# naver/dust3r

Hardware: NVIDIA H100
Metric: image-pairs/sec (512x384, ViT-L/B+DPT) (higher is better)
Workload: dtype bf16

## Files before the change

### dust3r_b200/csrc/attention_wgmma.cu

```cuda
#include "d3r_common.cuh"
#include "sm90_ptx.cuh"
#include "elementwise.h"
#include "prof.h"
#include "pdl.cuh"

namespace d3r {
namespace attn {

namespace wg {

constexpr int BQ = 128, BK = 128, D = 64;
constexpr int kThreads = 384;
constexpr int kTileBytes = 128 * 64 * 2;
constexpr int kPBytes = 2 * 64 * 128 * 2;
template <bool P_SMEM>
struct Smem {
  static constexpr int kP = P_SMEM ? 2 * kPBytes : 0;
  static constexpr int kBytes = kTileBytes  + 2 * kTileBytes  + 2 * kTileBytes  + kP + 128  + 1024;
  static_assert(kBytes <= 227 * 1024, "shared memory of one CTA");
};

template <bool P_SMEM>
__global__ void __launch_bounds__(kThreads, 1)
attention_kernel(const __grid_constant__ CUtensorMap tmap_q, const __grid_constant__ CUtensorMap tmap_k,
                 const __grid_constant__ CUtensorMap tmap_v, __nv_bfloat16* __restrict__ out, long long ldo, int Nq, int Nk,
                 int heads, int total_tiles, float scale_log2) {
  extern __shared__ uint8_t smem_raw[];
  uint8_t* smem = reinterpret_cast<uint8_t*>((reinterpret_cast<uintptr_t>(smem_raw) + 1023) & ~uintptr_t(1023));
  uint8_t* s_q = smem;
  uint8_t* s_k = s_q + kTileBytes;
  uint8_t* s_v = s_k + 2 * kTileBytes;
  uint8_t* s_p = s_v + 2 * kTileBytes;
  uint64_t* bars = reinterpret_cast<uint64_t*>(s_p + Smem<P_SMEM>::kP);
  uint64_t* q_full = bars + 0;
  uint64_t* q_empty = bars + 1;
  uint64_t* k_full = bars + 2;
  uint64_t* k_empty = bars + 4;
  uint64_t* v_full = bars + 6;
  uint64_t* v_empty = bars + 8;

  const int warp = threadIdx.x >> 5, lane = threadIdx.x & 31;
  const int nq_tiles = (Nq + BQ - 1) / BQ;
  const int nblk = (Nk + BK - 1) / BK;
  auto tile_coords = [&](int t, int& q0, int& h, int& b) {
    q0 = (t % nq_tiles) * BQ;
    h = (t / nq_tiles) % heads;
    b = t / (nq_tiles * heads);
  };

  if (threadIdx.x == 0) {
    ptx::prefetch_tmap(&tmap_q);
    ptx::prefetch_tmap(&tmap_k);
    ptx::prefetch_tmap(&tmap_v);
    ptx::mbar_init(ptx::smem_u32(q_full), 1);
    ptx::mbar_init(ptx::smem_u32(q_empty), 8);
    for (int s = 0; s < 2; ++s) {
      ptx::mbar_init(ptx::smem_u32(&k_full[s]), 1);
      ptx::mbar_init(ptx::smem_u32(&k_empty[s]), 8);
      ptx::mbar_init(ptx::smem_u32(&v_full[s]), 1);
      ptx::mbar_init(ptx::smem_u32(&v_empty[s]), 8);
    }
    ptx::fence_barrier_init();
  }
  __syncthreads();
  pdl::sync_with_predecessor();

  if (warp < 4) {
    ptx::setmaxnreg_dec<24>();
    if (warp == 0 && ptx::elect_one()) {
      uint32_t g = 0, it = 0;
      for (int t = blockIdx.x; t < total_tiles; t += gridDim.x, ++it) {
        int q0, h, b;
        tile_coords(t, q0, h, b);
        ptx::mbar_wait(ptx::smem_u32(q_empty), (it & 1) ^ 1);
        ptx::mbar_arrive_expect_tx(ptx::smem_u32(q_full), kTileBytes);
        ptx::tma_load_3d(ptx::smem_u32(s_q), &tmap_q, ptx::smem_u32(q_full), h * D, q0, b);
        for (int j = 0; j < nblk; ++j, ++g) {
          const int st = g & 1;
          const uint32_t ph = (g >> 1) & 1;
          ptx::mbar_wait(ptx::smem_u32(&k_empty[st]), ph ^ 1);
          ptx::mbar_arrive_expect_tx(ptx::smem_u32(&k_full[st]), kTileBytes);
          ptx::tma_load_3d(ptx::smem_u32(s_k + st * kTileBytes), &tmap_k, ptx::smem_u32(&k_full[st]), h * D, j * BK, b);
          ptx::mbar_wait(ptx::smem_u32(&v_empty[st]), ph ^ 1);
          ptx::mbar_arrive_expect_tx(ptx::smem_u32(&v_full[st]), kTileBytes);
          ptx::tma_load_3d(ptx::smem_u32(s_v + st * kTileBytes), &tmap_v, ptx::smem_u32(&v_full[st]), h * D, j * BK, b);
        }
      }
    }
  } else {
    ptx::setmaxnreg_inc<240>();
    const int cw = (threadIdx.x >> 7) - 1;
    const int wq = warp & 3, q = lane & 3;
    uint8_t* s_pw = s_p + cw * kPBytes;
    uint32_t g = 0, it = 0;
    for (int t = blockIdx.x; t < total_tiles; t += gridDim.x, ++it) {
      int q0, h, b;
      tile_coords(t, q0, h, b);
      float m_run[2] = {-INFINITY, -INFINITY}, l_run[2] = {0.f, 0.f};
      float o[32];
#pragma unroll
      for (int i = 0; i < 32; ++i) o[i] = 0.f;
      ptx::mbar_wait(ptx::smem_u32(q_full), it & 1);
      const uint64_t dq = ptx::desc_kmajor_sw128(ptx::smem_u32(s_q + cw * 64 * 128));
      for (int j = 0; j < nblk; ++j, ++g) {
        const int st = g & 1;
        const uint32_t ph = (g >> 1) & 1;
        float s[64];
        ptx::mbar_wait(ptx::smem_u32(&k_full[st]), ph);
        const uint64_t dk = ptx::desc_kmajor_sw128(ptx::smem_u32(s_k + st * kTileBytes));
        ptx::wgmma_fence();
#pragma unroll
        for (int k = 0; k < D / 16; ++k) ptx::wgmma_m64n128k16_ss(s, dq + uint64_t(2 * k), dk + uint64_t(2 * k), k ? 1u : 0u);
        ptx::wgmma_commit();
        ptx::wgmma_wait<0>();
        ptx::reg_fence(s);
        if (lane == 0) {
          ptx::mbar_arrive(ptx::smem_u32(&k_empty[st]));
          if (j == nblk - 1) ptx::mbar_arrive(ptx::smem_u32(q_empty));
        }
        const int nvalid = Nk - j * BK;
        if (nvalid < BK) {
#pragma unroll
          for (int n = 0; n < 16; ++n)
#pragma unroll
            for (int e = 0; e < 2; ++e)
              if (8 * n + 2 * q + e >= nvalid) { s[4 * n + e] = -INFINITY; s[4 * n + 2 + e] = -INFINITY; }
        }
        float ms[2];
#pragma unroll
        for (int hh = 0; hh < 2; ++hh) {
          float mx = -INFINITY;
#pragma unroll
          for (int n = 0; n < 16; ++n) mx = fmaxf(mx, fmaxf(s[4 * n + 2 * hh], s[4 * n + 2 * hh + 1]));
          mx = fmaxf(mx, __shfl_xor_sync(0xffffffffu, mx, 1));
          mx = fmaxf(mx, __shfl_xor_sync(0xffffffffu, mx, 2));
          const float m_new = fmaxf(m_run[hh], mx);
          const float corr = ptx::ex2_approx((m_run[hh] - m_new) * scale_log2);
          m_run[hh] = m_new;
          l_run[hh] *= corr;
#pragma unroll
          for (int n = 0; n < 8; ++n) { o[4 * n + 2 * hh] *= corr; o[4 * n + 2 * hh + 1] *= corr; }
          ms[hh] = m_new * scale_log2;
        }
        uint32_t pk[32];
#pragma unroll
        for (int n = 0; n < 16; ++n)
#pragma unroll
          for (int hh = 0; hh < 2; ++hh) {
            const float p0 = ptx::ex2_approx(fmaf(s[4 * n + 2 * hh], scale_log2, -ms[hh]));
            const float p1 = ptx::ex2_approx(fmaf(s[4 * n + 2 * hh + 1], scale_log2, -ms[hh]));
            l_run[hh] += p0 + p1;
            pk[2 * n + hh] = pack_bf16x2(p0, p1);
          }
        ptx::mbar_wait(ptx::smem_u32(&v_full[st]), ph);
        const uint32_t sv = ptx::smem_u32(s_v + st * kTileBytes);
        if constexpr (P_SMEM) {
#pragma unroll
          for (int n = 0; n < 16; ++n)
#pragma unroll
            for (int hh = 0; hh < 2; ++hh) {
              const int r = wq * 16 + (lane >> 2) + 8 * hh;
              *reinterpret_cast<uint32_t*>(s_pw + (n >> 3) * (64 * 128) + r * 128 + (((n & 7) ^ (r & 7)) << 4) + 4 * q) = pk[2 * n + hh];
            }
          ptx::fence_proxy_async();
          asm volatile("bar.sync %0, 128;" ::"r"(1 + cw) : "memory");
          const uint32_t sp = ptx::smem_u32(s_pw);
          ptx::wgmma_fence();
#pragma unroll
          for (int kk = 0; kk < BK / 16; ++kk)
            ptx::wgmma_m64n64k16_ss_tb(o, ptx::desc_kmajor_sw128(sp + (kk >> 2) * (64 * 128)) + uint64_t(2 * (kk & 3)),
                                       ptx::desc_mnmajor_sw128(sv + kk * 16 * 128), 1u);
        } else {
          ptx::wgmma_fence();
#pragma unroll
          for (int kk = 0; kk < BK / 16; ++kk) ptx::wgmma_m64n64k16_rs_tb(o, pk + 4 * kk, ptx::desc_mnmajor_sw128(sv + kk * 16 * 128), 1u);
        }
        ptx::wgmma_commit();
        ptx::wgmma_wait<0>();
        ptx::reg_fence(o);
        if constexpr (P_SMEM) asm volatile("bar.sync %0, 128;" ::"r"(1 + cw) : "memory");
        if (lane == 0) ptx::mbar_arrive(ptx::smem_u32(&v_empty[st]));
      }
#pragma unroll
      for (int hh = 0; hh < 2; ++hh) {
        float l = l_run[hh];
        l += __shfl_xor_sync(0xffffffffu, l, 1);
        l += __shfl_xor_sync(0xffffffffu, l, 2);
        const float inv = 1.f / l;
        const int qrow = q0 + cw * 64 + wq * 16 + (lane >> 2) + 8 * hh;
        if (qrow < Nq) {
          __nv_bfloat16* orow = out + ((long long)b * Nq + qrow) * ldo + h * D + 2 * q;
#pragma unroll
          for (int n = 0; n < 8; ++n)
            *reinterpret_cast<uint32_t*>(orow + 8 * n) = pack_bf16x2(o[4 * n + 2 * hh] * inv, o[4 * n + 2 * hh + 1] * inv);
        }
      }
    }
  }
}

}

template <bool P_SMEM>
static int launch_attention(const CUtensorMap& mq, const CUtensorMap& mk, const CUtensorMap& mv, void* out, long long ldo, int B, int heads,
                            int Nq, int Nk, float scale, cudaStream_t st) {
  static unsigned long long attr_devices = 0;
  if (first_launch_on_this_device(attr_devices))
    D3R_CUDA(cudaFuncSetAttribute(wg::attention_kernel<P_SMEM>, cudaFuncAttributeMaxDynamicSharedMemorySize, wg::Smem<P_SMEM>::kBytes));
  const int total_tiles = ((Nq + wg::BQ - 1) / wg::BQ) * heads * B;
  const int slots = num_sms();
  const int rounds = (total_tiles + slots - 1) / slots;
  const int grid = (total_tiles + rounds - 1) / rounds;
  prof::Scope scope(P_SMEM ? "attention_wgmma_psmem" : "attention_wgmma", st, 4.0 * double(B) * heads * double(Nq) * double(Nk) * 64.0);
  D3R_CUDA(pdl::launch(wg::attention_kernel<P_SMEM>, dim3(grid), dim3(wg::kThreads), size_t(wg::Smem<P_SMEM>::kBytes), st, mq, mk, mv,
                       (__nv_bfloat16*)out, ldo, Nq, Nk, heads, total_tiles, scale * 1.4426950408889634f));
  D3R_LAUNCH_CHECK();
  return D3R_OK;
}

static int make_map(CUtensorMap* m, const void* base, long long ld, int cols, int N, int B, int box_rows) {
  const cuuint64_t dims[3] = {(cuuint64_t)cols, (cuuint64_t)N, (cuuint64_t)B};
  const cuuint64_t str[2] = {(cuuint64_t)ld * 2, (cuuint64_t)N * ld * 2};
  const cuuint32_t box[3] = {64, (cuuint32_t)box_rows, 1};
  return encode_tensor_map(m, base, 3, dims, str, box, "attention");
}

static int g_impl = 3;

int attention_hd64(const void* q, long long ldq, const void* k, long long ldk, const void* v, long long ldv, void* out,
                   long long ldo, int B, int heads, int Nq, int Nk, float scale, cudaStream_t st) {
  D3R_CHECK_ARG(q && k && v && out && B > 0 && heads > 0 && Nq > 0 && Nk > 0, "attention: bad arguments");
  D3R_CHECK_ARG(ldq % 8 == 0 && ldk % 8 == 0 && ldv % 8 == 0 && ldo % 8 == 0, "attention: row strides must be multiples of 8");
  D3R_CHECK_ARG(((uintptr_t)q & 15) == 0 && ((uintptr_t)k & 15) == 0 && ((uintptr_t)v & 15) == 0 && ((uintptr_t)out & 15) == 0,
                "attention: pointers must be 16-byte aligned");
  CUtensorMap mq, mk, mv;
  int rc;
  if ((rc = make_map(&mq, q, ldq, heads * 64, Nq, B, wg::BQ))) return rc;
  if ((rc = make_map(&mk, k, ldk, heads * 64, Nk, B, wg::BK))) return rc;
  if ((rc = make_map(&mv, v, ldv, heads * 64, Nk, B, wg::BK))) return rc;
  if (g_impl == 2) return launch_attention<true>(mq, mk, mv, out, ldo, B, heads, Nq, Nk, scale, st);
  return launch_attention<false>(mq, mk, mv, out, ldo, B, heads, Nq, Nk, scale, st);
}

}
}

extern "C" void d3r_set_attention_impl(int32_t impl) { d3r::attn::g_impl = (impl == 2) ? 2 : 3; }

extern "C" int d3r_attention_hd64(const void* q, int64_t ldq, const void* k, int64_t ldk, const void* v, int64_t ldv, void* out,
                                  int64_t ldo, int32_t B, int32_t heads, int32_t Nq, int32_t Nk, float scale, void* stream) {
  return d3r::attn::attention_hd64(q, ldq, k, ldk, v, ldv, out, ldo, B, heads, Nq, Nk, scale, (cudaStream_t)stream);
}
```

### dust3r_b200/csrc/sm90_ptx.cuh

```cuda
#pragma once
#include <cuda.h>
#include <cuda_runtime.h>
#include <cuda_bf16.h>
#include <cstdint>

namespace d3r {
namespace ptx {

__device__ __forceinline__ uint32_t smem_u32(const void* p) { return static_cast<uint32_t>(__cvta_generic_to_shared(p)); }

__device__ __forceinline__ bool elect_one() {
  uint32_t pred = 0;
  asm volatile(
      "{\n"
      ".reg .b32 %%rx;\n"
      ".reg .pred %%px;\n"
      "elect.sync %%rx|%%px, %1;\n"
      "@%%px mov.s32 %0, 1;\n"
      "}\n"
      : "+r"(pred)
      : "r"(0xffffffffu));
  return pred != 0;
}

__device__ __forceinline__ void mbar_init(uint32_t bar, uint32_t count) {
  asm volatile("mbarrier.init.shared::cta.b64 [%0], %1;" ::"r"(bar), "r"(count));
}
__device__ __forceinline__ void fence_barrier_init() { asm volatile("fence.mbarrier_init.release.cluster;" ::: "memory"); }
__device__ __forceinline__ void fence_proxy_async() { asm volatile("fence.proxy.async.shared::cta;" ::: "memory"); }

__device__ __forceinline__ void mbar_arrive_expect_tx(uint32_t bar, uint32_t bytes) {
  asm volatile("mbarrier.arrive.expect_tx.shared::cta.b64 _, [%0], %1;" ::"r"(bar), "r"(bytes) : "memory");
}
__device__ __forceinline__ void mbar_arrive(uint32_t bar) {
  asm volatile("mbarrier.arrive.shared::cta.b64 _, [%0];" ::"r"(bar) : "memory");
}
__device__ __forceinline__ bool mbar_try_wait(uint32_t bar, uint32_t parity) {
  uint32_t done;
  asm volatile(
      "{\n"
      ".reg .pred p;\n"
      "mbarrier.try_wait.parity.shared::cta.b64 p, [%1], %2;\n"
      "selp.u32 %0, 1, 0, p;\n"
      "}\n"
      : "=r"(done)
      : "r"(bar), "r"(parity)
      : "memory");
  return done != 0;
}
__device__ __forceinline__ void mbar_wait(uint32_t bar, uint32_t parity) {
  while (!mbar_try_wait(bar, parity)) {
  }
}
__device__ __forceinline__ void mbar_wait_bounded(uint32_t bar, uint32_t parity) {
  uint32_t spins = 0;
  bool done;
  do {
    done = mbar_try_wait(bar, parity);
    if (!done && ++spins > (1u << 22)) __trap();
  } while (!done);
}

__device__ __forceinline__ void bulk_g2s(uint32_t dst, const void* src, uint32_t bytes, uint32_t bar) {
  asm volatile("cp.async.bulk.shared::cluster.global.mbarrier::complete_tx::bytes [%0], [%1], %2, [%3];"
               ::"r"(dst), "l"(src), "r"(bytes), "r"(bar) : "memory");
}
__device__ __forceinline__ uint64_t policy_evict_first() {
  uint64_t pol;
  asm volatile("createpolicy.fractional.L2::evict_first.b64 %0, 1.0;" : "=l"(pol));
  return pol;
}
__device__ __forceinline__ void bulk_g2s_hint(uint32_t dst, const void* src, uint32_t bytes, uint32_t bar, uint64_t pol) {
  asm volatile("cp.async.bulk.shared::cluster.global.mbarrier::complete_tx::bytes.L2::cache_hint [%0], [%1], %2, [%3], %4;"
               ::"r"(dst), "l"(src), "r"(bytes), "r"(bar), "l"(pol) : "memory");
}

__device__ __forceinline__ void prefetch_tmap(const void* tmap) {
  asm volatile("prefetch.tensormap [%0];" ::"l"(reinterpret_cast<uint64_t>(tmap)) : "memory");
}
__device__ __forceinline__ void tma_load_2d(uint32_t dst, const void* tmap, uint32_t bar, int c0, int c1) {
  asm volatile(
      "cp.async.bulk.tensor.2d.shared::cluster.global.mbarrier::complete_tx::bytes [%0], [%1, {%3, %4}], [%2];"
      ::"r"(dst), "l"(reinterpret_cast<uint64_t>(tmap)), "r"(bar), "r"(c0), "r"(c1)
      : "memory");
}
__device__ __forceinline__ void tma_load_3d(uint32_t dst, const void* tmap, uint32_t bar, int c0, int c1, int c2) {
  asm volatile(
      "cp.async.bulk.tensor.3d.shared::cluster.global.mbarrier::complete_tx::bytes [%0], [%1, {%3, %4, %5}], [%2];"
      ::"r"(dst), "l"(reinterpret_cast<uint64_t>(tmap)), "r"(bar), "r"(c0), "r"(c1), "r"(c2)
      : "memory");
}
__device__ __forceinline__ void tma_load_4d(uint32_t dst, const void* tmap, uint32_t bar, int c0, int c1, int c2, int c3) {
  asm volatile(
      "cp.async.bulk.tensor.4d.shared::cluster.global.mbarrier::complete_tx::bytes [%0], [%1, {%3, %4, %5, %6}], [%2];"
      ::"r"(dst), "l"(reinterpret_cast<uint64_t>(tmap)), "r"(bar), "r"(c0), "r"(c1), "r"(c2), "r"(c3)
      : "memory");
}
__device__ __forceinline__ void tma_load_3d_mc(uint32_t dst, const void* tmap, uint32_t bar, int c0, int c1, int c2, uint16_t mask) {
  asm volatile(
      "cp.async.bulk.tensor.3d.shared::cluster.global.mbarrier::complete_tx::bytes.multicast::cluster [%0], [%1, {%3, %4, %5}], [%2], %6;"
      ::"r"(dst), "l"(reinterpret_cast<uint64_t>(tmap)), "r"(bar), "r"(c0), "r"(c1), "r"(c2), "h"(mask)
      : "memory");
}

__device__ __forceinline__ void tma_store_2d(const void* tmap, uint32_t src, int c0, int c1) {
  asm volatile("cp.async.bulk.tensor.2d.global.shared::cta.tile.bulk_group [%0, {%2, %3}], [%1];"
               ::"l"(reinterpret_cast<uint64_t>(tmap)), "r"(src), "r"(c0), "r"(c1) : "memory");
}
__device__ __forceinline__ void tma_store_4d(const void* tmap, uint32_t src, int c0, int c1, int c2, int c3) {
  asm volatile("cp.async.bulk.tensor.4d.global.shared::cta.tile.bulk_group [%0, {%2, %3, %4, %5}], [%1];"
               ::"l"(reinterpret_cast<uint64_t>(tmap)), "r"(src), "r"(c0), "r"(c1), "r"(c2), "r"(c3) : "memory");
}
__device__ __forceinline__ void tma_reduce_add_2d(const void* tmap, uint32_t src, int c0, int c1) {
  asm volatile("cp.reduce.async.bulk.tensor.2d.global.shared::cta.add.tile.bulk_group [%0, {%2, %3}], [%1];"
               ::"l"(reinterpret_cast<uint64_t>(tmap)), "r"(src), "r"(c0), "r"(c1) : "memory");
}
__device__ __forceinline__ void bulk_commit_group() { asm volatile("cp.async.bulk.commit_group;" ::: "memory"); }
template <int N> __device__ __forceinline__ void bulk_wait_group_read() { asm volatile("cp.async.bulk.wait_group.read %0;" ::"n"(N) : "memory"); }
template <int N> __device__ __forceinline__ void bulk_wait_group() { asm volatile("cp.async.bulk.wait_group %0;" ::"n"(N) : "memory"); }
__device__ __forceinline__ void st_shared_b32(uint32_t addr, uint32_t v) { asm volatile("st.shared.b32 [%0], %1;" ::"r"(addr), "r"(v) : "memory"); }
__device__ __forceinline__ uint32_t ld_shared_b32(uint32_t addr) {
  uint32_t v;
  asm volatile("ld.shared.b32 %0, [%1];" : "=r"(v) : "r"(addr) : "memory");
  return v;
}
__device__ __forceinline__ void st_shared_v2_f32(uint32_t addr, float a, float b) {
  asm volatile("st.shared.v2.f32 [%0], {%1, %2};" ::"r"(addr), "f"(a), "f"(b) : "memory");
}
__device__ __forceinline__ void named_bar_sync(uint32_t id, uint32_t count) { asm volatile("bar.sync %0, %1;" ::"r"(id), "r"(count) : "memory"); }

__device__ __forceinline__ uint32_t cluster_ctarank() {
  uint32_t r;
  asm volatile("mov.u32 %0, %%cluster_ctarank;" : "=r"(r));
  return r;
}
__device__ __forceinline__ void cluster_sync() {
  asm volatile("barrier.cluster.arrive.release.aligned;\nbarrier.cluster.wait.acquire.aligned;" ::: "memory");
}
__device__ __forceinline__ void mbar_arrive_cluster(uint32_t bar, uint32_t rank) {
  asm volatile(
      "{\n"
      ".reg .b32 raddr;\n"
      "mapa.shared::cluster.u32 raddr, %0, %1;\n"
      "mbarrier.arrive.shared::cluster.b64 _, [raddr];\n"
      "}\n" ::"r"(bar), "r"(rank) : "memory");
}

__device__ __forceinline__ float ex2_approx(float x) { float y; asm("ex2.approx.ftz.f32 %0, %1;" : "=f"(y) : "f"(x)); return y; }
__device__ __forceinline__ float rcp_approx(float x) { float y; asm("rcp.approx.ftz.f32 %0, %1;" : "=f"(y) : "f"(x)); return y; }
__device__ __forceinline__ float rsqrt_approx(float x) { float y; asm("rsqrt.approx.ftz.f32 %0, %1;" : "=f"(y) : "f"(x)); return y; }
__device__ __forceinline__ float sqrt_approx(float x) { float y; asm("sqrt.approx.ftz.f32 %0, %1;" : "=f"(y) : "f"(x)); return y; }

template <int N> __device__ __forceinline__ void setmaxnreg_dec() { asm volatile("setmaxnreg.dec.sync.aligned.u32 %0;" ::"n"(N)); }
template <int N> __device__ __forceinline__ void setmaxnreg_inc() { asm volatile("setmaxnreg.inc.sync.aligned.u32 %0;" ::"n"(N)); }

__device__ __forceinline__ void wgmma_fence() { asm volatile("wgmma.fence.sync.aligned;" ::: "memory"); }
__device__ __forceinline__ void wgmma_commit() { asm volatile("wgmma.commit_group.sync.aligned;" ::: "memory"); }
template <int N> __device__ __forceinline__ void wgmma_wait() { asm volatile("wgmma.wait_group.sync.aligned %0;" ::"n"(N) : "memory"); }
template <int N> __device__ __forceinline__ void reg_fence(float (&d)[N]) {
#pragma unroll
  for (int i = 0; i < N; ++i) asm volatile("" : "+f"(d[i])::"memory");
}

__device__ __forceinline__ uint64_t desc_sw128(uint32_t smem_addr, uint32_t lbo_bytes) {
  uint64_t d = 0;
  d |= uint64_t((smem_addr & 0x3FFFF) >> 4);
  d |= uint64_t(lbo_bytes >> 4) << 16;
  d |= uint64_t(1024 >> 4) << 32;
  d |= uint64_t(1) << 62;
  return d;
}
__device__ __forceinline__ uint64_t desc_kmajor_sw128(uint32_t smem_addr) { return desc_sw128(smem_addr, 16); }
__device__ __forceinline__ uint64_t desc_mnmajor_sw128(uint32_t smem_addr) { return desc_sw128(smem_addr, 1024); }

__device__ __forceinline__ void wgmma_m64n64k16_ss(float* d, uint64_t desc_a, uint64_t desc_b, uint32_t accumulate) {
  asm volatile(
      "{\n"
      ".reg .pred p;\n"
      "setp.ne.b32 p, %34, 0;\n"
      "wgmma.mma_async.sync.aligned.m64n64k16.f32.bf16.bf16 "
      "{%0, %1, %2, %3, %4, %5, %6, %7, %8, %9, %10, %11, %12, %13, %14, %15, %16, %17, %18, %19, %20, %21, %22, %23, %24, %25, %26, %27, %28, %29, %30, %31}, %32, %33, p, 1, 1, 0, 0;\n"
      "}\n"
      : "+f"(d[0]), "+f"(d[1]), "+f"(d[2]), "+f"(d[3]), "+f"(d[4]), "+f"(d[5]), "+f"(d[6]), "+f"(d[7]), "+f"(d[8]), "+f"(d[9]), "+f"(d[10]), "+f"(d[11]), "+f"(d[12]), "+f"(d[13]), "+f"(d[14]), "+f"(d[15]), "+f"(d[16]), "+f"(d[17]), "+f"(d[18]), "+f"(d[19]), "+f"(d[20]), "+f"(d[21]), "+f"(d[22]), "+f"(d[23]), "+f"(d[24]), "+f"(d[25]), "+f"(d[26]), "+f"(d[27]), "+f"(d[28]), "+f"(d[29]), "+f"(d[30]), "+f"(d[31])
      : "l"(desc_a), "l"(desc_b), "r"(accumulate));
}
__device__ __forceinline__ void wgmma_m64n128k16_ss(float* d, uint64_t desc_a, uint64_t desc_b, uint32_t accumulate) {
  asm volatile(
      "{\n"
      ".reg .pred p;\n"
      "setp.ne.b32 p, %66, 0;\n"
      "wgmma.mma_async.sync.aligned.m64n128k16.f32.bf16.bf16 "
      "{%0, %1, %2, %3, %4, %5, %6, %7, %8, %9, %10, %11, %12, %13, %14, %15, %16, %17, %18, %19, %20, %21, %22, %23, %24, %25, %26, %27, %28, %29, %30, %31, %32, %33, %34, %35, %36, %37, %38, %39, %40, %41, %42, %43, %44, %45, %46, %47, %48, %49, %50, %51, %52, %53, %54, %55, %56, %57, %58, %59, %60, %61, %62, %63}, %64, %65, p, 1, 1, 0, 0;\n"
      "}\n"
      : "+f"(d[0]), "+f"(d[1]), "+f"(d[2]), "+f"(d[3]), "+f"(d[4]), "+f"(d[5]), "+f"(d[6]), "+f"(d[7]), "+f"(d[8]), "+f"(d[9]), "+f"(d[10]), "+f"(d[11]), "+f"(d[12]), "+f"(d[13]), "+f"(d[14]), "+f"(d[15]), "+f"(d[16]), "+f"(d[17]), "+f"(d[18]), "+f"(d[19]), "+f"(d[20]), "+f"(d[21]), "+f"(d[22]), "+f"(d[23]), "+f"(d[24]), "+f"(d[25]), "+f"(d[26]), "+f"(d[27]), "+f"(d[28]), "+f"(d[29]), "+f"(d[30]), "+f"(d[31]), "+f"(d[32]), "+f"(d[33]), "+f"(d[34]), "+f"(d[35]), "+f"(d[36]), "+f"(d[37]), "+f"(d[38]), "+f"(d[39]), "+f"(d[40]), "+f"(d[41]), "+f"(d[42]), "+f"(d[43]), "+f"(d[44]), "+f"(d[45]), "+f"(d[46]), "+f"(d[47]), "+f"(d[48]), "+f"(d[49]), "+f"(d[50]), "+f"(d[51]), "+f"(d[52]), "+f"(d[53]), "+f"(d[54]), "+f"(d[55]), "+f"(d[56]), "+f"(d[57]), "+f"(d[58]), "+f"(d[59]), "+f"(d[60]), "+f"(d[61]), "+f"(d[62]), "+f"(d[63])
      : "l"(desc_a), "l"(desc_b), "r"(accumulate));
}
__device__ __forceinline__ void wgmma_m64n256k16_ss(float* d, uint64_t desc_a, uint64_t desc_b, uint32_t accumulate) {
  asm volatile(
      "{\n"
      ".reg .pred p;\n"
      "setp.ne.b32 p, %130, 0;\n"
      "wgmma.mma_async.sync.aligned.m64n256k16.f32.bf16.bf16 "
      "{%0, %1, %2, %3, %4, %5, %6, %7, %8, %9, %10, %11, %12, %13, %14, %15, %16, %17, %18, %19, %20, %21, %22, %23, %24, %25, %26, %27, %28, %29, %30, %31, %32, %33, %34, %35, %36, %37, %38, %39, %40, %41, %42, %43, %44, %45, %46, %47, %48, %49, %50, %51, %52, %53, %54, %55, %56, %57, %58, %59, %60, %61, %62, %63, %64, %65, %66, %67, %68, %69, %70, %71, %72, %73, %74, %75, %76, %77, %78, %79, %80, %81, %82, %83, %84, %85, %86, %87, %88, %89, %90, %91, %92, %93, %94, %95, %96, %97, %98, %99, %100, %101, %102, %103, %104, %105, %106, %107, %108, %109, %110, %111, %112, %113, %114, %115, %116, %117, %118, %119, %120, %121, %122, %123, %124, %125, %126, %127}, %128, %129, p, 1, 1, 0, 0;\n"
      "}\n"
      : "+f"(d[0]), "+f"(d[1]), "+f"(d[2]), "+f"(d[3]), "+f"(d[4]), "+f"(d[5]), "+f"(d[6]), "+f"(d[7]), "+f"(d[8]), "+f"(d[9]), "+f"(d[10]), "+f"(d[11]), "+f"(d[12]), "+f"(d[13]), "+f"(d[14]), "+f"(d[15]), "+f"(d[16]), "+f"(d[17]), "+f"(d[18]), "+f"(d[19]), "+f"(d[20]), "+f"(d[21]), "+f"(d[22]), "+f"(d[23]), "+f"(d[24]), "+f"(d[25]), "+f"(d[26]), "+f"(d[27]), "+f"(d[28]), "+f"(d[29]), "+f"(d[30]), "+f"(d[31]), "+f"(d[32]), "+f"(d[33]), "+f"(d[34]), "+f"(d[35]), "+f"(d[36]), "+f"(d[37]), "+f"(d[38]), "+f"(d[39]), "+f"(d[40]), "+f"(d[41]), "+f"(d[42]), "+f"(d[43]), "+f"(d[44]), "+f"(d[45]), "+f"(d[46]), "+f"(d[47]), "+f"(d[48]), "+f"(d[49]), "+f"(d[50]), "+f"(d[51]), "+f"(d[52]), "+f"(d[53]), "+f"(d[54]), "+f"(d[55]), "+f"(d[56]), "+f"(d[57]), "+f"(d[58]), "+f"(d[59]), "+f"(d[60]), "+f"(d[61]), "+f"(d[62]), "+f"(d[63]), "+f"(d[64]), "+f"(d[65]), "+f"(d[66]), "+f"(d[67]), "+f"(d[68]), "+f"(d[69]), "+f"(d[70]), "+f"(d[71]), "+f"(d[72]), "+f"(d[73]), "+f"(d[74]), "+f"(d[75]), "+f"(d[76]), "+f"(d[77]), "+f"(d[78]), "+f"(d[79]), "+f"(d[80]), "+f"(d[81]), "+f"(d[82]), "+f"(d[83]), "+f"(d[84]), "+f"(d[85]), "+f"(d[86]), "+f"(d[87]), "+f"(d[88]), "+f"(d[89]), "+f"(d[90]), "+f"(d[91]), "+f"(d[92]), "+f"(d[93]), "+f"(d[94]), "+f"(d[95]), "+f"(d[96]), "+f"(d[97]), "+f"(d[98]), "+f"(d[99]), "+f"(d[100]), "+f"(d[101]), "+f"(d[102]), "+f"(d[103]), "+f"(d[104]), "+f"(d[105]), "+f"(d[106]), "+f"(d[107]), "+f"(d[108]), "+f"(d[109]), "+f"(d[110]), "+f"(d[111]), "+f"(d[112]), "+f"(d[113]), "+f"(d[114]), "+f"(d[115]), "+f"(d[116]), "+f"(d[117]), "+f"(d[118]), "+f"(d[119]), "+f"(d[120]), "+f"(d[121]), "+f"(d[122]), "+f"(d[123]), "+f"(d[124]), "+f"(d[125]), "+f"(d[126]), "+f"(d[127])
      : "l"(desc_a), "l"(desc_b), "r"(accumulate));
}
__device__ __forceinline__ void wgmma_m64n64k16_rs_tb(float* d, const uint32_t* a, uint64_t desc_b, uint32_t accumulate) {
  asm volatile(
      "{\n"
      ".reg .pred p;\n"
      "setp.ne.b32 p, %37, 0;\n"
      "wgmma.mma_async.sync.aligned.m64n64k16.f32.bf16.bf16 "
      "{%0, %1, %2, %3, %4, %5, %6, %7, %8, %9, %10, %11, %12, %13, %14, %15, %16, %17, %18, %19, %20, %21, %22, %23, %24, %25, %26, %27, %28, %29, %30, %31}, {%32, %33, %34, %35}, %36, p, 1, 1, 1;\n"
      "}\n"
      : "+f"(d[0]), "+f"(d[1]), "+f"(d[2]), "+f"(d[3]), "+f"(d[4]), "+f"(d[5]), "+f"(d[6]), "+f"(d[7]), "+f"(d[8]), "+f"(d[9]), "+f"(d[10]), "+f"(d[11]), "+f"(d[12]), "+f"(d[13]), "+f"(d[14]), "+f"(d[15]), "+f"(d[16]), "+f"(d[17]), "+f"(d[18]), "+f"(d[19]), "+f"(d[20]), "+f"(d[21]), "+f"(d[22]), "+f"(d[23]), "+f"(d[24]), "+f"(d[25]), "+f"(d[26]), "+f"(d[27]), "+f"(d[28]), "+f"(d[29]), "+f"(d[30]), "+f"(d[31])
      : "r"(a[0]), "r"(a[1]), "r"(a[2]), "r"(a[3]), "l"(desc_b), "r"(accumulate));
}
__device__ __forceinline__ void wgmma_m64n64k16_ss_tb(float* d, uint64_t desc_a, uint64_t desc_b, uint32_t accumulate) {
  asm volatile(
      "{\n"
      ".reg .pred p;\n"
      "setp.ne.b32 p, %34, 0;\n"
      "wgmma.mma_async.sync.aligned.m64n64k16.f32.bf16.bf16 "
      "{%0, %1, %2, %3, %4, %5, %6, %7, %8, %9, %10, %11, %12, %13, %14, %15, %16, %17, %18, %19, %20, %21, %22, %23, %24, %25, %26, %27, %28, %29, %30, %31}, %32, %33, p, 1, 1, 0, 1;\n"
      "}\n"
      : "+f"(d[0]), "+f"(d[1]), "+f"(d[2]), "+f"(d[3]), "+f"(d[4]), "+f"(d[5]), "+f"(d[6]), "+f"(d[7]), "+f"(d[8]), "+f"(d[9]), "+f"(d[10]), "+f"(d[11]), "+f"(d[12]), "+f"(d[13]), "+f"(d[14]), "+f"(d[15]), "+f"(d[16]), "+f"(d[17]), "+f"(d[18]), "+f"(d[19]), "+f"(d[20]), "+f"(d[21]), "+f"(d[22]), "+f"(d[23]), "+f"(d[24]), "+f"(d[25]), "+f"(d[26]), "+f"(d[27]), "+f"(d[28]), "+f"(d[29]), "+f"(d[30]), "+f"(d[31])
      : "l"(desc_a), "l"(desc_b), "r"(accumulate));
}

}
}
```

Measured before the change: 232.8.

## Rewrite default attention kernel as FA3-style ping-pong with intra-warpgroup overlap

The default register-P attention path becomes a new kernel with one TMA producer warpgroup and three consumer warpgroups handling 192 query rows. It uses double-buffered Q slots and a 3-stage K/V ring. Consumers take turns issuing WGMMAs through named barriers, so one warpgroup's softmax overlaps another's tensor-core work. Within a warpgroup, the next block's QK^T is issued alongside the previous block's PV, so softmax also overlaps matmul. The cost is higher register pressure per consumer, a 192-row tile that changes tile counts and wave quantization, and more intricate barrier and phase logic.

Result: faster. 237.4 (median of 6 runs) (+2.0%).

```diff
diff --git a/dust3r_b200/csrc/attention_wgmma.cu b/dust3r_b200/csrc/attention_wgmma.cu
--- a/dust3r_b200/csrc/attention_wgmma.cu
+++ b/dust3r_b200/csrc/attention_wgmma.cu
@@ -13,25 +13,23 @@
 constexpr int kThreads = 384;
 constexpr int kTileBytes = 128 * 64 * 2;
 constexpr int kPBytes = 2 * 64 * 128 * 2;
-template <bool P_SMEM>
-struct Smem {
-  static constexpr int kP = P_SMEM ? 2 * kPBytes : 0;
-  static constexpr int kBytes = kTileBytes  + 2 * kTileBytes  + 2 * kTileBytes  + kP + 128  + 1024;
+
+struct SmemPsmem {
+  static constexpr int kBytes = kTileBytes  + 2 * kTileBytes  + 2 * kTileBytes  + 2 * kPBytes + 128  + 1024;
   static_assert(kBytes <= 227 * 1024, "shared memory of one CTA");
 };
 
-template <bool P_SMEM>
 __global__ void __launch_bounds__(kThreads, 1)
-attention_kernel(const __grid_constant__ CUtensorMap tmap_q, const __grid_constant__ CUtensorMap tmap_k,
-                 const __grid_constant__ CUtensorMap tmap_v, __nv_bfloat16* __restrict__ out, long long ldo, int Nq, int Nk,
-                 int heads, int total_tiles, float scale_log2) {
+attention_psmem_kernel(const __grid_constant__ CUtensorMap tmap_q, const __grid_constant__ CUtensorMap tmap_k,
+                       const __grid_constant__ CUtensorMap tmap_v, __nv_bfloat16* __restrict__ out, long long ldo, int Nq, int Nk,
+                       int heads, int total_tiles, float scale_log2) {
   extern __shared__ uint8_t smem_raw[];
   uint8_t* smem = reinterpret_cast<uint8_t*>((reinterpret_cast<uintptr_t>(smem_raw) + 1023) & ~uintptr_t(1023));
   uint8_t* s_q = smem;
   uint8_t* s_k = s_q + kTileBytes;
   uint8_t* s_v = s_k + 2 * kTileBytes;
   uint8_t* s_p = s_v + 2 * kTileBytes;
-  uint64_t* bars = reinterpret_cast<uint64_t*>(s_p + Smem<P_SMEM>::kP);
+  uint64_t* bars = reinterpret_cast<uint64_t*>(s_p + 2 * kPBytes);
   uint64_t* q_full = bars + 0;
   uint64_t* q_empty = bars + 1;
   uint64_t* k_full = bars + 2;
@@ -154,31 +152,25 @@
           }
         ptx::mbar_wait(ptx::smem_u32(&v_full[st]), ph);
         const uint32_t sv = ptx::smem_u32(s_v + st * kTileBytes);
-        if constexpr (P_SMEM) {
-#pragma unroll
-          for (int n = 0; n < 16; ++n)
-#pragma unroll
-            for (int hh = 0; hh < 2; ++hh) {
-              const int r = wq * 16 + (lane >> 2) + 8 * hh;
-              *reinterpret_cast<uint32_t*>(s_pw + (n >> 3) * (64 * 128) + r * 128 + (((n & 7) ^ (r & 7)) << 4) + 4 * q) = pk[2 * n + hh];
-            }
-          ptx::fence_proxy_async();
-          asm volatile("bar.sync %0, 128;" ::"r"(1 + cw) : "memory");
-          const uint32_t sp = ptx::smem_u32(s_pw);
-          ptx::wgmma_fence();
-#pragma unroll
-          for (int kk = 0; kk < BK / 16; ++kk)
-            ptx::wgmma_m64n64k16_ss_tb(o, ptx::desc_kmajor_sw128(sp + (kk >> 2) * (64 * 128)) + uint64_t(2 * (kk & 3)),
-                                       ptx::desc_mnmajor_sw128(sv + kk * 16 * 128), 1u);
-        } else {
-          ptx::wgmma_fence();
-#pragma unroll
-          for (int kk = 0; kk < BK / 16; ++kk) ptx::wgmma_m64n64k16_rs_tb(o, pk + 4 * kk, ptx::desc_mnmajor_sw128(sv + kk * 16 * 128), 1u);
-        }
+#pragma unroll
+        for (int n = 0; n < 16; ++n)
+#pragma unroll
+          for (int hh = 0; hh < 2; ++hh) {
+            const int r = wq * 16 + (lane >> 2) + 8 * hh;
+            *reinterpret_cast<uint32_t*>(s_pw + (n >> 3) * (64 * 128) + r * 128 + (((n & 7) ^ (r & 7)) << 4) + 4 * q) = pk[2 * n + hh];
+          }
+        ptx::fence_proxy_async();
+        asm volatile("bar.sync %0, 128;" ::"r"(1 + cw) : "memory");
+        const uint32_t sp = ptx::smem_u32(s_pw);
+        ptx::wgmma_fence();
+#pragma unroll
+        for (int kk = 0; kk < BK / 16; ++kk)
+          ptx::wgmma_m64n64k16_ss_tb(o, ptx::desc_kmajor_sw128(sp + (kk >> 2) * (64 * 128)) + uint64_t(2 * (kk & 3)),
+                                     ptx::desc_mnmajor_sw128(sv + kk * 16 * 128), 1u);
         ptx::wgmma_commit();
         ptx::wgmma_wait<0>();
         ptx::reg_fence(o);
-        if constexpr (P_SMEM) asm volatile("bar.sync %0, 128;" ::"r"(1 + cw) : "memory");
+        asm volatile("bar.sync %0, 128;" ::"r"(1 + cw) : "memory");
         if (lane == 0) ptx::mbar_arrive(ptx::smem_u32(&v_empty[st]));
       }
 #pragma unroll
@@ -199,20 +191,252 @@
   }
 }
 
+constexpr int kConsumers = 3, kQRows = 64 * kConsumers, kPpThreads = 128 * (1 + kConsumers);
+constexpr int kQTileBytes = kQRows * 128;
+constexpr int kQSlots = 2, kKvStages = 3;
+constexpr int kBarTurn = 3;
+struct Smem {
+  static constexpr int kBytes = kQSlots * kQTileBytes + 2 * kKvStages * kTileBytes  + 128  + 1024;
+  static_assert(kBytes <= 227 * 1024, "shared memory of one CTA");
+};
+
+__global__ void __launch_bounds__(kPpThreads, 1)
+attention_kernel(const __grid_constant__ CUtensorMap tmap_q, const __grid_constant__ CUtensorMap tmap_k,
+                 const __grid_constant__ CUtensorMap tmap_v, __nv_bfloat16* __restrict__ out, long long ldo, int Nq, int Nk,
+                 int heads, int total_tiles, float scale_log2) {
+  extern __shared__ uint8_t smem_raw[];
+  uint8_t* smem = reinterpret_cast<uint8_t*>((reinterpret_cast<uintptr_t>(smem_raw) + 1023) & ~uintptr_t(1023));
+  uint8_t* s_q = smem;
+  uint8_t* s_k = s_q + kQSlots * kQTileBytes;
+  uint8_t* s_v = s_k + kKvStages * kTileBytes;
+  uint64_t* bars = reinterpret_cast<uint64_t*>(s_v + kKvStages * kTileBytes);
+  uint64_t* q_full = bars + 0;
+  uint64_t* q_empty = q_full + kQSlots;
+  uint64_t* k_full = q_empty + kQSlots;
+  uint64_t* k_empty = k_full + kKvStages;
+  uint64_t* v_full = k_empty + kKvStages;
+  uint64_t* v_empty = v_full + kKvStages;
+  auto slot = [](uint32_t u, uint32_t n) { return u % n; };
+  auto parity = [](uint32_t u, uint32_t n) { return (u / n) & 1u; };
+
+  const int warp = threadIdx.x >> 5, lane = threadIdx.x & 31;
+  const int nq_tiles = (Nq + kQRows - 1) / kQRows;
+  const int nblk = (Nk + BK - 1) / BK;
+  auto tile_coords = [&](int t, int& q0, int& h, int& b) {
+    q0 = (t % nq_tiles) * kQRows;
+    h = (t / nq_tiles) % heads;
+    b = t / (nq_tiles * heads);
+  };
+
+  if (threadIdx.x == 0) {
+    ptx::prefetch_tmap(&tmap_q);
+    ptx::prefetch_tmap(&tmap_k);
+    ptx::prefetch_tmap(&tmap_v);
+    for (int s = 0; s < kQSlots; ++s) {
+      ptx::mbar_init(ptx::smem_u32(&q_full[s]), 1);
+      ptx::mbar_init(ptx::smem_u32(&q_empty[s]), 4 * kConsumers);
+    }
+    for (int s = 0; s < kKvStages; ++s) {
+      ptx::mbar_init(ptx::smem_u32(&k_full[s]), 1);
+      ptx::mbar_init(ptx::smem_u32(&k_empty[s]), 4 * kConsumers);
+      ptx::mbar_init(ptx::smem_u32(&v_full[s]), 1);
+      ptx::mbar_init(ptx::smem_u32(&v_empty[s]), 4 * kConsumers);
+    }
+    ptx::fence_barrier_init();
+  }
+  __syncthreads();
+  pdl::sync_with_predecessor();
+
+  if (warp < 4) {
+    ptx::setmaxnreg_dec<24>();
+    if (warp == 0 && ptx::elect_one()) {
+      uint32_t g = 0, it = 0;
+      for (int t = blockIdx.x; t < total_tiles; t += gridDim.x, ++it) {
+        int q0, h, b;
+        tile_coords(t, q0, h, b);
+        const uint32_t qs = slot(it, kQSlots);
+        ptx::mbar_wait(ptx::smem_u32(&q_empty[qs]), parity(it, kQSlots) ^ 1);
+        ptx::mbar_arrive_expect_tx(ptx::smem_u32(&q_full[qs]), kQTileBytes);
+        ptx::tma_load_3d(ptx::smem_u32(s_q + qs * kQTileBytes), &tmap_q, ptx::smem_u32(&q_full[qs]), h * D, q0, b);
+        for (int j = 0; j < nblk; ++j, ++g) {
+          const uint32_t st = slot(g, kKvStages), ph = parity(g, kKvStages);
+          ptx::mbar_wait(ptx::smem_u32(&k_empty[st]), ph ^ 1);
+          ptx::mbar_arrive_expect_tx(ptx::smem_u32(&k_full[st]), kTileBytes);
+          ptx::tma_load_3d(ptx::smem_u32(s_k + st * kTileBytes), &tmap_k, ptx::smem_u32(&k_full[st]), h * D, j * BK, b);
+          ptx::mbar_wait(ptx::smem_u32(&v_empty[st]), ph ^ 1);
+          ptx::mbar_arrive_expect_tx(ptx::smem_u32(&v_full[st]), kTileBytes);
+          ptx::tma_load_3d(ptx::smem_u32(s_v + st * kTileBytes), &tmap_v, ptx::smem_u32(&v_full[st]), h * D, j * BK, b);
+        }
+      }
+    }
+  } else {
+    ptx::setmaxnreg_inc<160>();
+    const int cw = (threadIdx.x >> 7) - 1;
+    const int wq = warp & 3, q = lane & 3;
+    const uint32_t my_turn = kBarTurn + cw, other_turn = kBarTurn + (cw + 1) % kConsumers;
+    if (cw == kConsumers - 1) ptx::named_bar_arrive(kBarTurn, 256);
+    float s[64], o[32], corr[2];
+    uint32_t pk[32];
+    uint32_t g = 0, it = 0;
+
+    auto wait_full = [&](uint64_t* bar, uint32_t blk) { ptx::mbar_wait(ptx::smem_u32(&bar[slot(blk, kKvStages)]), parity(blk, kKvStages)); };
+    auto issue_s = [&](uint64_t dq, uint32_t blk) {
+      const uint32_t st = slot(blk, kKvStages);
+      const uint64_t dk = ptx::desc_kmajor_sw128(ptx::smem_u32(s_k + st * kTileBytes));
+#pragma unroll
+      for (int k = 0; k < D / 16; ++k) ptx::wgmma_m64n128k16_ss(s, dq + uint64_t(2 * k), dk + uint64_t(2 * k), k ? 1u : 0u);
+      ptx::wgmma_commit();
+    };
+    auto issue_pv = [&](uint32_t blk) {
+      const uint32_t st = slot(blk, kKvStages);
+      const uint32_t sv = ptx::smem_u32(s_v + st * kTileBytes);
+#pragma unroll
+      for (int kk = 0; kk < BK / 16; ++kk) ptx::wgmma_m64n64k16_rs_tb(o, pk + 4 * kk, ptx::desc_mnmajor_sw128(sv + kk * 16 * 128), 1u);
+      ptx::wgmma_commit();
+    };
+    auto release = [&](uint64_t* bar, uint32_t blk) {
+      if (lane == 0) ptx::mbar_arrive(ptx::smem_u32(&bar[slot(blk, kKvStages)]));
+    };
+    auto softmax = [&](int j, float (&m_run)[2], float (&l_run)[2]) {
+      const int nvalid = Nk - j * BK;
+      if (nvalid < BK) {
+#pragma unroll
+        for (int n = 0; n < 16; ++n)
+#pragma unroll
+          for (int e = 0; e < 2; ++e)
+            if (8 * n + 2 * q + e >= nvalid) { s[4 * n + e] = -INFINITY; s[4 * n + 2 + e] = -INFINITY; }
+      }
+      float ms[2];
+#pragma unroll
+      for (int hh = 0; hh < 2; ++hh) {
+        float mx = -INFINITY;
+#pragma unroll
+        for (int n = 0; n < 16; ++n) mx = fmaxf(mx, fmaxf(s[4 * n + 2 * hh], s[4 * n + 2 * hh + 1]));
+        mx = fmaxf(mx, __shfl_xor_sync(0xffffffffu, mx, 1));
+        mx = fmaxf(mx, __shfl_xor_sync(0xffffffffu, mx, 2));
+        const float m_new = fmaxf(m_run[hh], mx);
+        corr[hh] = ptx::ex2_approx((m_run[hh] - m_new) * scale_log2);
+        m_run[hh] = m_new;
+        l_run[hh] *= corr[hh];
+        ms[hh] = m_new * scale_log2;
+      }
+#pragma unroll
+      for (int n = 0; n < 16; ++n)
+#pragma unroll
+        for (int hh = 0; hh < 2; ++hh) {
+          const float p0 = ptx::ex2_approx(fmaf(s[4 * n + 2 * hh], scale_log2, -ms[hh]));
+          const float p1 = ptx::ex2_approx(fmaf(s[4 * n + 2 * hh + 1], scale_log2, -ms[hh]));
+          l_run[hh] += p0 + p1;
+          s[4 * n + 2 * hh] = p0;
+          s[4 * n + 2 * hh + 1] = p1;
+        }
+    };
+    auto rescale = [&]() {
+#pragma unroll
+      for (int hh = 0; hh < 2; ++hh)
+#pragma unroll
+        for (int n = 0; n < 8; ++n) { o[4 * n + 2 * hh] *= corr[hh]; o[4 * n + 2 * hh + 1] *= corr[hh]; }
+    };
+    auto pack = [&]() {
+#pragma unroll
+      for (int n = 0; n < 16; ++n)
+#pragma unroll
+        for (int hh = 0; hh < 2; ++hh) pk[2 * n + hh] = pack_bf16x2(s[4 * n + 2 * hh], s[4 * n + 2 * hh + 1]);
+    };
+
+    for (int t = blockIdx.x; t < total_tiles; t += gridDim.x, ++it) {
+      int q0, h, b;
+      tile_coords(t, q0, h, b);
+      float m_run[2] = {-INFINITY, -INFINITY}, l_run[2] = {0.f, 0.f};
+#pragma unroll
+      for (int i = 0; i < 32; ++i) o[i] = 0.f;
+      const uint32_t qs = slot(it, kQSlots);
+      ptx::mbar_wait(ptx::smem_u32(&q_full[qs]), parity(it, kQSlots));
+      const uint64_t dq = ptx::desc_kmajor_sw128(ptx::smem_u32(s_q + qs * kQTileBytes + cw * 64 * 128));
+      auto release_q = [&]() {
+        if (lane == 0) ptx::mbar_arrive(ptx::smem_u32(&q_empty[qs]));
+      };
+
+      ptx::named_bar_sync(my_turn, 256);
+      wait_full(k_full, g);
+      ptx::wgmma_fence();
+      issue_s(dq, g);
+      ptx::named_bar_arrive(other_turn, 256);
+      ptx::wgmma_wait<0>();
+      ptx::reg_fence(s);
+      release(k_empty, g);
+      if (nblk == 1) release_q();
+      softmax(0, m_run, l_run);
+      for (int j = 1; j < nblk; ++j) {
+        ptx::wgmma_wait<0>();
+        ptx::reg_fence(o);
+        ptx::reg_fence(s);
+        if (j >= 2) release(v_empty, g + j - 2);
+        rescale();
+        pack();
+        ptx::named_bar_sync(my_turn, 256);
+        wait_full(k_full, g + j);
+        wait_full(v_full, g + j - 1);
+        ptx::wgmma_fence();
+        issue_s(dq, g + j);
+        issue_pv(g + j - 1);
+        ptx::named_bar_arrive(other_turn, 256);
+        ptx::wgmma_wait<1>();
+        ptx::reg_fence(s);
+        release(k_empty, g + j);
+        if (j == nblk - 1) release_q();
+        softmax(j, m_run, l_run);
+      }
+      ptx::wgmma_wait<0>();
+      ptx::reg_fence(o);
+      ptx::reg_fence(s);
+      if (nblk >= 2) release(v_empty, g + nblk - 2);
+      rescale();
+      pack();
+      wait_full(v_full, g + nblk - 1);
+      ptx::wgmma_fence();
+      issue_pv(g + nblk - 1);
+      ptx::wgmma_wait<0>();
+      ptx::reg_fence(o);
+      release(v_empty, g + nblk - 1);
+      g += nblk;
+
+#pragma unroll
+      for (int hh = 0; hh < 2; ++hh) {
+        float l = l_run[hh];
+        l += __shfl_xor_sync(0xffffffffu, l, 1);
+        l += __shfl_xor_sync(0xffffffffu, l, 2);
+        const float inv = 1.f / l;
+        const int qrow = q0 + cw * 64 + wq * 16 + (lane >> 2) + 8 * hh;
+        if (qrow < Nq) {
+          __nv_bfloat16* orow = out + ((long long)b * Nq + qrow) * ldo + h * D + 2 * q;
+#pragma unroll
+          for (int n = 0; n < 8; ++n)
+            *reinterpret_cast<uint32_t*>(orow + 8 * n) = pack_bf16x2(o[4 * n + 2 * hh] * inv, o[4 * n + 2 * hh + 1] * inv);
+        }
+      }
+    }
+    if (cw == 0) ptx::named_bar_sync(my_turn, 256);
+  }
+}
+
 }
 
 template <bool P_SMEM>
 static int launch_attention(const CUtensorMap& mq, const CUtensorMap& mk, const CUtensorMap& mv, void* out, long long ldo, int B, int heads,
                             int Nq, int Nk, float scale, cudaStream_t st) {
+  auto* kernel = P_SMEM ? wg::attention_psmem_kernel : wg::attention_kernel;
+  const int smem_bytes = P_SMEM ? wg::SmemPsmem::kBytes : wg::Smem::kBytes;
+  const int bq = P_SMEM ? wg::BQ : wg::kQRows, threads = P_SMEM ? wg::kThreads : wg::kPpThreads;
   static unsigned long long attr_devices = 0;
   if (first_launch_on_this_device(attr_devices))
-    D3R_CUDA(cudaFuncSetAttribute(wg::attention_kernel<P_SMEM>, cudaFuncAttributeMaxDynamicSharedMemorySize, wg::Smem<P_SMEM>::kBytes));
-  const int total_tiles = ((Nq + wg::BQ - 1) / wg::BQ) * heads * B;
+    D3R_CUDA(cudaFuncSetAttribute(kernel, cudaFuncAttributeMaxDynamicSharedMemorySize, smem_bytes));
+  const int total_tiles = ((Nq + bq - 1) / bq) * heads * B;
   const int slots = num_sms();
   const int rounds = (total_tiles + slots - 1) / slots;
   const int grid = (total_tiles + rounds - 1) / rounds;
   prof::Scope scope(P_SMEM ? "attention_wgmma_psmem" : "attention_wgmma", st, 4.0 * double(B) * heads * double(Nq) * double(Nk) * 64.0);
-  D3R_CUDA(pdl::launch(wg::attention_kernel<P_SMEM>, dim3(grid), dim3(wg::kThreads), size_t(wg::Smem<P_SMEM>::kBytes), st, mq, mk, mv,
+  D3R_CUDA(pdl::launch(kernel, dim3(grid), dim3(threads), size_t(smem_bytes), st, mq, mk, mv,
                        (__nv_bfloat16*)out, ldo, Nq, Nk, heads, total_tiles, scale * 1.4426950408889634f));
   D3R_LAUNCH_CHECK();
   return D3R_OK;
@@ -235,7 +459,7 @@
                 "attention: pointers must be 16-byte aligned");
   CUtensorMap mq, mk, mv;
   int rc;
-  if ((rc = make_map(&mq, q, ldq, heads * 64, Nq, B, wg::BQ))) return rc;
+  if ((rc = make_map(&mq, q, ldq, heads * 64, Nq, B, g_impl == 2 ? wg::BQ : wg::kQRows))) return rc;
   if ((rc = make_map(&mk, k, ldk, heads * 64, Nk, B, wg::BK))) return rc;
   if ((rc = make_map(&mv, v, ldv, heads * 64, Nk, B, wg::BK))) return rc;
   if (g_impl == 2) return launch_attention<true>(mq, mk, mv, out, ldo, B, heads, Nq, Nk, scale, st);
diff --git a/dust3r_b200/csrc/sm90_ptx.cuh b/dust3r_b200/csrc/sm90_ptx.cuh
--- a/dust3r_b200/csrc/sm90_ptx.cuh
+++ b/dust3r_b200/csrc/sm90_ptx.cuh
@@ -128,6 +128,7 @@
   asm volatile("st.shared.v2.f32 [%0], {%1, %2};" ::"r"(addr), "f"(a), "f"(b) : "memory");
 }
 __device__ __forceinline__ void named_bar_sync(uint32_t id, uint32_t count) { asm volatile("bar.sync %0, %1;" ::"r"(id), "r"(count) : "memory"); }
+__device__ __forceinline__ void named_bar_arrive(uint32_t id, uint32_t count) { asm volatile("bar.arrive %0, %1;" ::"r"(id), "r"(count) : "memory"); }
 
 __device__ __forceinline__ uint32_t cluster_ctarank() {
   uint32_t r;
```
